# zju3dv/OnePose_Plus_Plus

Hardware: AMD Instinct MI355X
Metric: query images/sec (2D-3D match fwd) at 512x512 img x 5k pts (higher is better)
Workload: dtype f32 (operands as exact bf16 triples, f32 accumulate)

## Files before the change

onepose_plus_plus_amd/csrc/enc_layer64.hip:

```cpp
#include <stdlib.h>

#include <type_traits>

#include "enc_frag.h"

namespace {

constexpr int R64 = 64, C = 256, NW = 8, NT = 512, D = 32;
constexpr int SA = a_stride_bytes(C);
constexpr int SS = C + 4;
constexpr int OFF_S = R64 * SA, OFF_Z = OFF_S + 32 * SS * 4;
constexpr size_t kLds64 = OFF_Z + 1024;

__global__ __launch_bounds__(NT) void enc_layer64_kernel(const OppEncChain a) {
  extern __shared__ __attribute__((aligned(16))) char smem[];
  char* A = smem;
  float* S = reinterpret_cast<float*>(smem + OFF_S);
  float* z_sh = reinterpret_cast<float*>(smem + OFF_Z);

  const int tid = threadIdx.x, lane = tid & 63;
  const int wave = __builtin_amdgcn_readfirstlane(tid >> 6);
  const int half = lane >> 5, l31 = lane & 31;

  const int chunks0 = (a.len0 + R64 - 1) / R64;
  const int stream = (int)blockIdx.x >= chunks0 ? 1 : 0;
  const int cidx = stream ? blockIdx.x - chunks0 : blockIdx.x;
  const int seg_len = stream ? a.len1 : a.len0;
  const int row0 = (stream ? a.len0 : 0) + cidx * R64;
  const int nrows = min(R64, seg_len - cidx * R64);
  const float* qrows = (stream && a.q1 != nullptr) ? a.q1 + (size_t)(cidx * R64) * a.ldq : a.q + (size_t)row0 * a.ldq;

  const char* a_lane = A + l31 * SA + half * 48;
  auto gemm = [&](auto ntile_c, auto depth_c, auto s0_c, auto s1_c, auto ks_c, const void* wf, int t0, f32x16 (&acc)[2][decltype(ntile_c)::value], int tstep = 1) {
    constexpr int NTILE = decltype(ntile_c)::value, DEPTH = decltype(depth_c)::value;
    constexpr int S0 = decltype(s0_c)::value, S1 = decltype(s1_c)::value, KS = decltype(ks_c)::value;
    constexpr int NSTEP = S1 - S0;
    const __amdgpu_buffer_rsrc_t rsrc = __builtin_amdgcn_make_buffer_rsrc(const_cast<void*>(wf), 0, 0x7fffffff, 0x00020000);
    const int voff = lane * 16;
    u32x4 bq[DEPTH][NTILE][3];
    u32x4 af[2][2][3];
    auto load_b = [&](int s, int slot) {
#pragma unroll
      for (int j = 0; j < NTILE; ++j)
#pragma unroll
        for (int p = 0; p < 3; ++p)
          bq[slot][j][p] = __builtin_amdgcn_raw_buffer_load_b128(rsrc, voff, (((t0 + j * tstep) * KS + S0 + s) * 3 + p) * 1024, 0);
    };
    auto load_a = [&](int s, int slot) {
#pragma unroll
      for (int i = 0; i < 2; ++i)
#pragma unroll
        for (int q = 0; q < 3; ++q) af[slot][i][q] = *reinterpret_cast<const u32x4*>(a_lane + i * 32 * SA + s * 96 + q * 16);
    };
#pragma unroll
    for (int s = 0; s < DEPTH && s < NSTEP; ++s) load_b(s, s);
    load_a(0, 0);
    __builtin_amdgcn_sched_barrier(0);
    constexpr int PA[6] = {2, 0, 1, 1, 0, 0};
    constexpr int PB[6] = {0, 2, 1, 0, 1, 0};
#pragma unroll
    for (int s = 0; s < NSTEP; ++s) {
      if (s + 1 < NSTEP) load_a(s + 1, (s + 1) & 1);
#pragma unroll
      for (int pr = 0; pr < 6; ++pr)
#pragma unroll
        for (int i = 0; i < 2; ++i)
#pragma unroll
          for (int j = 0; j < NTILE; ++j)
            acc[i][j] = __builtin_amdgcn_mfma_f32_32x32x16_bf16(__builtin_bit_cast(bf16x8, af[s & 1][i][PA[pr]]),
                                                                 __builtin_bit_cast(bf16x8, bq[s % DEPTH][j][PB[pr]]), acc[i][j], 0, 0, 0);
      if (s + DEPTH < NSTEP) load_b(s + DEPTH, s % DEPTH);
      __builtin_amdgcn_sched_barrier(0);
    }
  };
  auto ic = [](auto v) { return v; };
  (void)ic;
  auto stage = [&](const f32x16& t, int col0, bool relu) {
#pragma unroll
    for (int r = 0; r < 16; ++r) {
      const int row = (r & 3) + 8 * (r >> 2) + 4 * half;
      float v = t[r];
      if (relu) v = v < 0.f ? 0.f : v;
      S[row * SS + col0 + l31] = v;
    }
  };
  auto split_staged = [&](int rb, int g0) {
#pragma unroll
    for (int i = 0; i < 32 * (C / 8) / NT; ++i) {
      const int p = tid + i * NT;
      const int r = p / (C / 8), g = p - r * (C / 8);
      const float4* s4 = reinterpret_cast<const float4*>(S + r * SS + g * 8);
      split8_store(s4[0], s4[1], A + (rb + r) * SA + (g0 + g) * 48);
    }
  };
  typedef float vec_t __attribute__((ext_vector_type(4)));
  auto layernorm_rows = [&](const float* gamma, const float* beta, float eps, auto mode_c, int rb) {
    constexpr int MODE = decltype(mode_c)::value;
    const vec_t gmv = *reinterpret_cast<const vec_t*>(gamma + lane * 4);
    const vec_t btv = *reinterpret_cast<const vec_t*>(beta + lane * 4);
    constexpr int RPW = 32 / NW;
    float v[RPW][4], sm[RPW], mean[RPW], rstd[RPW];
#pragma unroll
    for (int r = 0; r < RPW; ++r) {
      const vec_t t = *reinterpret_cast<const vec_t*>(S + (wave * RPW + r) * SS + lane * 4);
      sm[r] = 0.f;
#pragma unroll
      for (int i = 0; i < 4; ++i) {
        v[r][i] = t[i];
        sm[r] += t[i];
      }
    }
#pragma unroll
    for (int r = 0; r < RPW; ++r) sm[r] = opp_wave_sum_dpp(sm[r]);
#pragma unroll
    for (int r = 0; r < RPW; ++r) {
      mean[r] = sm[r] / (float)C;
      sm[r] = 0.f;
#pragma unroll
      for (int i = 0; i < 4; ++i) {
        const float d = v[r][i] - mean[r];
        sm[r] = opp_ln_sq_acc(d, sm[r]);
      }
    }
#pragma unroll
    for (int r = 0; r < RPW; ++r) sm[r] = opp_wave_sum_dpp(sm[r]);
#pragma unroll
    for (int r = 0; r < RPW; ++r) rstd[r] = 1.0f / sqrtf(sm[r] / (float)C + eps);
#pragma unroll
    for (int r = 0; r < RPW; ++r) {
      const int lr = rb + wave * RPW + r;
      float y[4];
#pragma unroll
      for (int i = 0; i < 4; ++i) y[i] = opp_ln_affine(v[r][i], mean[r], rstd[r], gmv[i], btv[i]);
      if constexpr (MODE != 0) {
        if (lr < nrows) {
          const vec_t xr = *reinterpret_cast<const vec_t*>(a.X + (size_t)(row0 + lr) * a.ldx + lane * 4);
          vec_t o;
#pragma unroll
          for (int i = 0; i < 4; ++i) o[i] = xr[i] + y[i];
          *reinterpret_cast<vec_t*>(a.out + (size_t)(row0 + lr) * a.ldo + lane * 4) = o;
#pragma unroll
          for (int i = 0; i < 4; ++i) y[i] = o[i];
        } else {
#pragma unroll
          for (int i = 0; i < 4; ++i) y[i] = 0.f;
        }
      }
      if constexpr (MODE != 1) {
        char* g = A + lr * SA + ((lane * 4) >> 3) * 48 + ((lane * 4) & 7) * 2;
#pragma unroll
        for (int i = 0; i < 4; i += 2) {
          unsigned hi, mid, lo;
          split2(y[i], y[i + 1], hi, mid, lo);
          *reinterpret_cast<unsigned*>(g + i * 2) = hi;
          *reinterpret_cast<unsigned*>(g + 16 + i * 2) = mid;
          *reinterpret_cast<unsigned*>(g + 32 + i * 2) = lo;
        }
      }
    }
  };
  auto zero2 = [](auto& acc) {
#pragma unroll
    for (auto& row : acc)
#pragma unroll
      for (auto& t : row)
#pragma unroll
        for (int r = 0; r < 16; ++r) t[r] = 0.f;
  };
  using I0 = std::integral_constant<int, 0>;
  using I1 = std::integral_constant<int, 1>;
  using I2 = std::integral_constant<int, 2>;
  using I3 = std::integral_constant<int, 3>;
  using I4 = std::integral_constant<int, 4>;
  using I16 = std::integral_constant<int, 16>;
  using I32 = std::integral_constant<int, 32>;

#pragma unroll
  for (int i = 0; i < R64 * (C / 8) / NT; ++i) {
    const int p = tid + i * NT;
    const int r = p / (C / 8), g = p - r * (C / 8);
    float4 v0 = make_float4(0.f, 0.f, 0.f, 0.f), v1 = v0;
    if (r < nrows) {
      const float4* s4 = reinterpret_cast<const float4*>(a.X + (size_t)(row0 + r) * a.ldx + g * 8);
      v0 = s4[0];
      v1 = s4[1];
    }
    split8_store(v0, v1, A + r * SA + g * 48);
  }
  const int src = a.cross ? 1 - stream : stream;
  const float src_len = (float)(src ? a.len1 : a.len0);
  const float* kvp = (src && a.kv1 != nullptr) ? a.kv1 : a.kv + (size_t)src * (C * D);
  const float* ksp = (src && a.ks1 != nullptr) ? a.ks1 : a.ks + (size_t)src * C;
  const int h = wave;
  float bk[16];
#pragma unroll
  for (int i = 0; i < 16; ++i) bk[i] = kvp[(h * D + 2 * i + half) * D + l31];
  __syncthreads();
  f32x16 hid[2][2];
  zero2(hid);
  gemm(I2{}, I3{}, I0{}, I16{}, I32{}, a.w1, wave * 2, hid);
  __syncthreads();

  constexpr int QS = 258;
  float* qsh = S;
#pragma unroll
  for (int rh = 0; rh < 2; ++rh) {
#pragma unroll
    for (int i = 0; i < 32 * (C / 4) / NT; ++i) {
      const int e = tid + i * NT;
      const int r = e / (C / 4), c4 = e - r * (C / 4);
      float4 q = make_float4(0.f, 0.f, 0.f, 0.f);
      if (rh * 32 + r < nrows) q = *reinterpret_cast<const float4*>(qrows + (size_t)(rh * 32 + r) * a.ldq + c4 * 4);
      float2* dst = reinterpret_cast<float2*>(qsh + r * QS + c4 * 4);
      dst[0] = make_float2(q.x, q.y);
      dst[1] = make_float2(q.z, q.w);
    }
    __syncthreads();
    if (tid < 8 * 32) {
      const int tok = tid & 31, hh = tid >> 5;
      const float* q = qsh + tok * QS + hh * D;
      const float* k = ksp + hh * D;
      float den = 0.f;
#pragma unroll
      for (int d = 0; d < D; ++d) den = fmaf(q[d], k[d], den);
      z_sh[hh * 32 + tok] = 1.0f / (den + a.eps_attn);
    }
    f32x16 num;
#pragma unroll
    for (int r = 0; r < 16; ++r) num[r] = 0.f;
#pragma unroll
    for (int i = 0; i < 16; ++i) num = __builtin_amdgcn_mfma_f32_32x32x2f32(qsh[l31 * QS + h * D + 2 * i + half], bk[i], num, 0, 0, 0);
    __syncthreads();
    {
      char* col = A + (h * 4 + (l31 >> 3)) * 48 + (l31 & 7) * 2;
#pragma unroll
      for (int r = 0; r < 16; ++r) {
        const int row = (r & 3) + 8 * (r >> 2) + 4 * half;
        const float v = (num[r] * z_sh[h * 32 + row]) * src_len;
        unsigned hi, mid, lo;
        split2(v, 0.f, hi, mid, lo);
        char* d = col + (rh * 32 + row) * SA;
        *reinterpret_cast<unsigned short*>(d) = (unsigned short)hi;
        *reinterpret_cast<unsigned short*>(d + 16) = (unsigned short)mid;
        *reinterpret_cast<unsigned short*>(d + 32) = (unsigned short)lo;
      }
    }
    __syncthreads();
  }

  {
    f32x16 acc[2][1];
    zero2(acc);
    gemm(I1{}, I4{}, I0{}, I16{}, I16{}, a.wm, wave, acc);
    __syncthreads();
#pragma unroll
    for (int rh = 0; rh < 2; ++rh) {
      stage(acc[rh][0], wave * 32, false);
      __syncthreads();
      layernorm_rows(a.g1, a.b1, a.eps_ln, I0{}, rh * 32);
      __syncthreads();
    }
  }

  gemm(I2{}, I3{}, I16{}, I32{}, I32{}, a.w1, wave * 2, hid);
  __syncthreads();

  f32x16 out[2][1];
  zero2(out);
#pragma unroll
  for (int kh = 0; kh < 2; ++kh) {
#pragma unroll
    for (int rh = 0; rh < 2; ++rh) {
      if (wave / (NW / 2) == kh) {
        const int c0 = (wave - kh * (NW / 2)) * 64;
        stage(hid[rh][0], c0, true);
        stage(hid[rh][1], c0 + 32, true);
      }
      __syncthreads();
      split_staged(rh * 32, 0);
      __syncthreads();
    }
    if (kh == 0) gemm(I1{}, I4{}, I0{}, I16{}, I32{}, a.w2, wave, out);
    else gemm(I1{}, I4{}, I16{}, I32{}, I32{}, a.w2, wave, out);
    __syncthreads();
  }

  const bool fold = a.wq_next != nullptr;
#pragma unroll
  for (int rh = 0; rh < 2; ++rh) {
    stage(out[rh][0], wave * 32, false);
    __syncthreads();
    if (fold) layernorm_rows(a.g2, a.b2, a.eps_ln, I2{}, rh * 32);
    else layernorm_rows(a.g2, a.b2, a.eps_ln, I1{}, rh * 32);
    __syncthreads();
  }
  if (!fold) return;

  float* qdst = (stream && a.qkv_out1 != nullptr) ? a.qkv_out1 + (size_t)(cidx * R64) * (3 * C) : a.qkv_out + (size_t)row0 * (3 * C);
  const float vdiv = (float)seg_len;
  auto finish_qkv = [&](f32x16& t, int rb, bool qk) {
#pragma unroll
    for (int r = 0; r < 16; ++r) {
      const int row = rb + (r & 3) + 8 * (r >> 2) + 4 * half;
      float v = 0.f;
      if (row < nrows) {
        v = t[r];
        if (qk) v = v > 0.f ? v + 1.f : __expf(v);
        else v = v / vdiv;
        if (stream == 0 && a.qmask != nullptr) v *= a.qmask[row0 + row];
      }
      t[r] = v;
    }
  };
  auto store_qkv = [&](const f32x16& t, int rb, int tile) {
    const int col = tile * 32 + l31;
#pragma unroll
    for (int r = 0; r < 16; ++r) {
      const int row = rb + (r & 3) + 8 * (r >> 2) + 4 * half;
      if (row < nrows) qdst[(size_t)row * (3 * C) + col] = t[r];
    }
  };
  const bool kv_fold = a.kv_part != nullptr;
  {
    f32x16 acc[2][1];
    zero2(acc);
    gemm(I1{}, I4{}, I0{}, I16{}, I16{}, a.wq_next, h, acc);
#pragma unroll
    for (int i = 0; i < 2; ++i) {
      finish_qkv(acc[i][0], i * 32, true);
      store_qkv(acc[i][0], i * 32, h);
    }
  }
  f32x16 acc[2][2];
  zero2(acc);
  gemm(I2{}, I3{}, I0{}, I16{}, I16{}, a.wq_next, NW + h, acc, NW);
#pragma unroll
  for (int i = 0; i < 2; ++i) {
    finish_qkv(acc[i][0], i * 32, true);
    finish_qkv(acc[i][1], i * 32, false);
  }
  if (!kv_fold) {
#pragma unroll
    for (int i = 0; i < 2; ++i) {
      store_qkv(acc[i][0], i * 32, NW + h);
      store_qkv(acc[i][1], i * 32, 2 * NW + h);
    }
    return;
  }
  {
    f32x16 kvacc;
#pragma unroll
    for (int r = 0; r < 16; ++r) kvacc[r] = 0.f;
    float ksum = 0.f;
    auto swap = [](float x, float y, float& lo, float& hi) {
      const auto r = __builtin_amdgcn_permlane32_swap(__builtin_bit_cast(unsigned, x), __builtin_bit_cast(unsigned, y), false, false);
      lo = __builtin_bit_cast(float, (unsigned)r[0]);
      hi = __builtin_bit_cast(float, (unsigned)r[1]);
    };
#pragma unroll
    for (int i = 0; i < 2; ++i)
#pragma unroll
      for (int q = 0; q < 4; ++q) {
        float kk[2][2], vv[2][2];
#pragma unroll
        for (int e = 0; e < 2; ++e) {
          swap(acc[i][0][4 * q + 2 * e], acc[i][0][4 * q + 2 * e + 1], kk[0][e], kk[1][e]);
          swap(acc[i][1][4 * q + 2 * e], acc[i][1][4 * q + 2 * e + 1], vv[0][e], vv[1][e]);
        }
#pragma unroll
        for (int g = 0; g < 2; ++g)
#pragma unroll
          for (int e = 0; e < 2; ++e) {
            kvacc = __builtin_amdgcn_mfma_f32_32x32x2f32(kk[g][e], vv[g][e], kvacc, 0, 0, 0);
            ksum += kk[g][e];
          }
      }
    float* kvp = a.kv_part + (size_t)blockIdx.x * (C * D) + h * (D * D);
#pragma unroll
    for (int r = 0; r < 16; ++r) {
      const int d = (r & 3) + 8 * (r >> 2) + 4 * half;
      kvp[d * D + l31] = kvacc[r];
    }
    const float tot = ksum + __shfl_xor(ksum, 32, 64);
    if (half == 0) a.ks_part[(size_t)blockIdx.x * C + h * D + l31] = tot;
  }
}

}

int opp_enc_layer64(const OppEncChain& a, hipStream_t stream) {
  OPP_CHECK_ARG(a.C == 256 && a.apply && a.X && a.out && a.q && a.kv && a.ks && a.wm && a.w1 && a.w2 && a.g1 && a.b1 && a.g2 && a.b2,
                "enc_layer64: coarse level (C = 256) with the fused attention apply only");
  OPP_CHECK_ARG(a.len0 >= 0 && a.len1 >= 0 && a.len0 + a.len1 > 0, "enc_layer64: empty token set");
  auto al16 = [](const void* p) { return (reinterpret_cast<uintptr_t>(p) & 15) == 0; };
  OPP_CHECK_ARG(al16(a.X) && al16(a.out) && al16(a.q) && a.ldx % 4 == 0 && a.ldo % 4 == 0 && a.ldq % 4 == 0 && al16(a.g1) && al16(a.b1) &&
                    al16(a.g2) && al16(a.b2) && al16(a.wm) && al16(a.w1) && al16(a.w2) && al16(a.q1), "enc_layer64: operands must be 16-byte aligned");
  OPP_CHECK_ARG(a.wq_next == nullptr || (a.qkv_out != nullptr && al16(a.wq_next)), "enc_layer64: folded projection needs its output buffer");
  OPP_CHECK_ARG((a.kv_part == nullptr) == (a.ks_part == nullptr) && (a.kv_part == nullptr || (a.wq_next != nullptr && a.qkv_out1 == nullptr)),
                "enc_layer64: the KV partials need the folded projection and both of their buffers");
  static OppLdsOnce lds_once;
  opp_lds_opt_in(reinterpret_cast<const void*>(enc_layer64_kernel), kLds64, lds_once);
  const int tiles = opp_cdiv(a.len0, R64) + opp_cdiv(a.len1, R64);
  OppProfScope prof(OPP_PROF_ENC_CHAIN, stream, 2.0 * (double)(a.len0 + a.len1) * ((a.wq_next ? 10.0 : 7.0) * C * C + 32.0 * C));
  hipLaunchKernelGGL(enc_layer64_kernel, dim3(tiles), dim3(NT), kLds64, stream, a);
  OPP_CHECK_LAUNCH("enc_layer64_kernel");
  return OPP_OK;
}
```

Baseline: 586.5.

## Keep attention message and FFN hidden in registers, cut block barriers in encoder layer

After: 586.8, median of 2. Within noise of the previous version (+0.0%).

```diff
diff --git a/onepose_plus_plus_amd/csrc/enc_layer64.hip b/onepose_plus_plus_amd/csrc/enc_layer64.hip
--- a/onepose_plus_plus_amd/csrc/enc_layer64.hip
+++ b/onepose_plus_plus_amd/csrc/enc_layer64.hip
@@ -12,7 +12,9 @@
 constexpr int OFF_S = R64 * SA, OFF_Z = OFF_S + 32 * SS * 4;
 constexpr size_t kLds64 = OFF_Z + 1024;
 
-__global__ __launch_bounds__(NT) void enc_layer64_kernel(const OppEncChain a) {
+constexpr int kStampSlots = 16, kStamps = 14;
+template <bool STAMP>
+__device__ __forceinline__ void enc_layer64_body(const OppEncChain& a, unsigned long long* ts_out) {
   extern __shared__ __attribute__((aligned(16))) char smem[];
   char* A = smem;
   float* S = reinterpret_cast<float*>(smem + OFF_S);
@@ -21,6 +23,20 @@
   const int tid = threadIdx.x, lane = tid & 63;
   const int wave = __builtin_amdgcn_readfirstlane(tid >> 6);
   const int half = lane >> 5, l31 = lane & 31;
+  unsigned long long ts[kStamps] = {};
+  auto stamp = [&](int i) {
+    if constexpr (STAMP) ts[i] = __builtin_readcyclecounter();
+  };
+  auto flush_stamps = [&]() {
+    if constexpr (STAMP) {
+      if (lane == 0) {
+        unsigned long long* o = ts_out + ((size_t)blockIdx.x * NW + wave) * kStampSlots;
+#pragma unroll
+        for (int i = 0; i < kStamps; ++i) o[i] = ts[i];
+      }
+    }
+  };
+  stamp(0);
 
   const int chunks0 = (a.len0 + R64 - 1) / R64;
   const int stream = (int)blockIdx.x >= chunks0 ? 1 : 0;
@@ -31,7 +47,7 @@
   const float* qrows = (stream && a.q1 != nullptr) ? a.q1 + (size_t)(cidx * R64) * a.ldq : a.q + (size_t)row0 * a.ldq;
 
   const char* a_lane = A + l31 * SA + half * 48;
-  auto gemm = [&](auto ntile_c, auto depth_c, auto s0_c, auto s1_c, auto ks_c, const void* wf, int t0, f32x16 (&acc)[2][decltype(ntile_c)::value], int tstep = 1) {
+  auto gemm = [&](auto ntile_c, auto depth_c, auto s0_c, auto s1_c, auto ks_c, const void* wf, int t0, f32x16 (&acc)[2][decltype(ntile_c)::value], auto&& tail, int tstep = 1) {
     constexpr int NTILE = decltype(ntile_c)::value, DEPTH = decltype(depth_c)::value;
     constexpr int S0 = decltype(s0_c)::value, S1 = decltype(s1_c)::value, KS = decltype(ks_c)::value;
     constexpr int NSTEP = S1 - S0;
@@ -70,30 +86,51 @@
             acc[i][j] = __builtin_amdgcn_mfma_f32_32x32x16_bf16(__builtin_bit_cast(bf16x8, af[s & 1][i][PA[pr]]),
                                                                  __builtin_bit_cast(bf16x8, bq[s % DEPTH][j][PB[pr]]), acc[i][j], 0, 0, 0);
       if (s + DEPTH < NSTEP) load_b(s + DEPTH, s % DEPTH);
+      if (s + DEPTH == NSTEP) tail();
       __builtin_amdgcn_sched_barrier(0);
     }
   };
-  auto ic = [](auto v) { return v; };
-  (void)ic;
-  auto stage = [&](const f32x16& t, int col0, bool relu) {
+  auto none = [] {};
+  auto stage = [&](const f32x16& t, int col0) {
 #pragma unroll
     for (int r = 0; r < 16; ++r) {
       const int row = (r & 3) + 8 * (r >> 2) + 4 * half;
-      float v = t[r];
-      if (relu) v = v < 0.f ? 0.f : v;
-      S[row * SS + col0 + l31] = v;
-    }
-  };
-  auto split_staged = [&](int rb, int g0) {
-#pragma unroll
-    for (int i = 0; i < 32 * (C / 8) / NT; ++i) {
-      const int p = tid + i * NT;
-      const int r = p / (C / 8), g = p - r * (C / 8);
-      const float4* s4 = reinterpret_cast<const float4*>(S + r * SS + g * 8);
-      split8_store(s4[0], s4[1], A + (rb + r) * SA + (g0 + g) * 48);
-    }
+      S[row * SS + col0 + l31] = t[r];
+    }
+  };
+  auto acc_to_operand = [&](const f32x16& t, int rb, int c0) {
+    const int odd = l31 & 1;
+    char* base = A + (rb + 4 * half + odd) * SA + ((c0 + l31) >> 3) * 48 + (l31 & 6) * 2;
+#pragma unroll
+    for (int r = 0; r < 16; r += 2) {
+      const float e = t[r], o = t[r + 1];
+      const float got = __builtin_bit_cast(float, __builtin_amdgcn_update_dpp(0, __builtin_bit_cast(int, odd ? +e : +o), 0xB1, 0xF, 0xF, true));
+      unsigned hi, mid, lo;
+      split2(odd ? +got : +e, odd ? +o : +got, hi, mid, lo);
+      char* d = base + ((r & 3) + 8 * (r >> 2)) * SA;
+      *reinterpret_cast<unsigned*>(d) = hi;
+      *reinterpret_cast<unsigned*>(d + 16) = mid;
+      *reinterpret_cast<unsigned*>(d + 32) = lo;
+    }
+  };
+  auto relu16 = [](const f32x16& t) {
+    f32x16 o;
+#pragma unroll
+    for (int r = 0; r < 16; ++r) o[r] = t[r] < 0.f ? 0.f : t[r];
+    return o;
   };
   typedef float vec_t __attribute__((ext_vector_type(4)));
+  vec_t xres[2][32 / NW];
+  auto load_x_rows = [&]() {
+#pragma unroll
+    for (int rh = 0; rh < 2; ++rh)
+#pragma unroll
+      for (int r = 0; r < 32 / NW; ++r) {
+        const int lr = rh * 32 + wave * (32 / NW) + r;
+        xres[rh][r] = vec_t{0.f, 0.f, 0.f, 0.f};
+        if (lr < nrows) xres[rh][r] = *reinterpret_cast<const vec_t*>(a.X + (size_t)(row0 + lr) * a.ldx + lane * 4);
+      }
+  };
   auto layernorm_rows = [&](const float* gamma, const float* beta, float eps, auto mode_c, int rb) {
     constexpr int MODE = decltype(mode_c)::value;
     const vec_t gmv = *reinterpret_cast<const vec_t*>(gamma + lane * 4);
@@ -134,7 +171,7 @@
       for (int i = 0; i < 4; ++i) y[i] = opp_ln_affine(v[r][i], mean[r], rstd[r], gmv[i], btv[i]);
       if constexpr (MODE != 0) {
         if (lr < nrows) {
-          const vec_t xr = *reinterpret_cast<const vec_t*>(a.X + (size_t)(row0 + lr) * a.ldx + lane * 4);
+          const vec_t xr = xres[rb / 32][r];
           vec_t o;
 #pragma unroll
           for (int i = 0; i < 4; ++i) o[i] = xr[i] + y[i];
@@ -175,17 +212,24 @@
   using I16 = std::integral_constant<int, 16>;
   using I32 = std::integral_constant<int, 32>;
 
-#pragma unroll
-  for (int i = 0; i < R64 * (C / 8) / NT; ++i) {
-    const int p = tid + i * NT;
-    const int r = p / (C / 8), g = p - r * (C / 8);
-    float4 v0 = make_float4(0.f, 0.f, 0.f, 0.f), v1 = v0;
-    if (r < nrows) {
-      const float4* s4 = reinterpret_cast<const float4*>(a.X + (size_t)(row0 + r) * a.ldx + g * 8);
-      v0 = s4[0];
-      v1 = s4[1];
-    }
-    split8_store(v0, v1, A + r * SA + g * 48);
+  {
+    constexpr int XI = R64 * (C / 8) / NT;
+    float4 xv[XI][2];
+#pragma unroll
+    for (int i = 0; i < XI; ++i) {
+      const int p = tid + i * NT;
+      const int r = p / (C / 8), g = p - r * (C / 8);
+      const float4* s4 = reinterpret_cast<const float4*>(a.X + (size_t)(row0 + min(r, nrows - 1)) * a.ldx + g * 8);
+      xv[i][0] = s4[0];
+      xv[i][1] = s4[1];
+    }
+#pragma unroll
+    for (int i = 0; i < XI; ++i) {
+      const int p = tid + i * NT;
+      const int r = p / (C / 8), g = p - r * (C / 8);
+      const float4 zero = make_float4(0.f, 0.f, 0.f, 0.f);
+      split8_store(r < nrows ? xv[i][0] : zero, r < nrows ? xv[i][1] : zero, A + r * SA + g * 48);
+    }
   }
   const int src = a.cross ? 1 - stream : stream;
   const float src_len = (float)(src ? a.len1 : a.len0);
@@ -196,105 +240,116 @@
 #pragma unroll
   for (int i = 0; i < 16; ++i) bk[i] = kvp[(h * D + 2 * i + half) * D + l31];
   __syncthreads();
+  stamp(1);
+  auto load_q = [&](int rh, float4 (&q)[8]) {
+    const float4* p = reinterpret_cast<const float4*>(qrows + (size_t)min(rh * 32 + l31, nrows - 1) * a.ldq + h * D);
+#pragma unroll
+    for (int i = 0; i < 8; ++i) q[i] = p[i];
+  };
+  float4 qv0[8];
   f32x16 hid[2][2];
   zero2(hid);
-  gemm(I2{}, I3{}, I0{}, I16{}, I32{}, a.w1, wave * 2, hid);
+  gemm(I2{}, I3{}, I0{}, I16{}, I32{}, a.w1, wave * 2, hid, [&] { load_q(0, qv0); });
   __syncthreads();
-
-  constexpr int QS = 258;
-  float* qsh = S;
+  stamp(2);
+
+  float4 qv1[8];
+  load_q(1, qv1);
 #pragma unroll
   for (int rh = 0; rh < 2; ++rh) {
-#pragma unroll
-    for (int i = 0; i < 32 * (C / 4) / NT; ++i) {
-      const int e = tid + i * NT;
-      const int r = e / (C / 4), c4 = e - r * (C / 4);
-      float4 q = make_float4(0.f, 0.f, 0.f, 0.f);
-      if (rh * 32 + r < nrows) q = *reinterpret_cast<const float4*>(qrows + (size_t)(rh * 32 + r) * a.ldq + c4 * 4);
-      float2* dst = reinterpret_cast<float2*>(qsh + r * QS + c4 * 4);
-      dst[0] = make_float2(q.x, q.y);
-      dst[1] = make_float2(q.z, q.w);
-    }
-    __syncthreads();
-    if (tid < 8 * 32) {
-      const int tok = tid & 31, hh = tid >> 5;
-      const float* q = qsh + tok * QS + hh * D;
-      const float* k = ksp + hh * D;
+    float q[D];
+#pragma unroll
+    for (int i = 0; i < 8; ++i) {
+      float4 t = qv0[i];
+      if (rh) t = qv1[i];
+      if (rh * 32 + l31 >= nrows) t = make_float4(0.f, 0.f, 0.f, 0.f);
+      q[4 * i] = t.x, q[4 * i + 1] = t.y, q[4 * i + 2] = t.z, q[4 * i + 3] = t.w;
+    }
+    {
+      const float* k = ksp + h * D;
       float den = 0.f;
 #pragma unroll
       for (int d = 0; d < D; ++d) den = fmaf(q[d], k[d], den);
-      z_sh[hh * 32 + tok] = 1.0f / (den + a.eps_attn);
-    }
+      z_sh[h * 32 + l31] = 1.0f / (den + a.eps_attn);
+    }
+    __builtin_amdgcn_fence(__ATOMIC_RELEASE, "wavefront");
+    __builtin_amdgcn_wave_barrier();
+    __builtin_amdgcn_fence(__ATOMIC_ACQUIRE, "wavefront");
     f32x16 num;
 #pragma unroll
     for (int r = 0; r < 16; ++r) num[r] = 0.f;
 #pragma unroll
-    for (int i = 0; i < 16; ++i) num = __builtin_amdgcn_mfma_f32_32x32x2f32(qsh[l31 * QS + h * D + 2 * i + half], bk[i], num, 0, 0, 0);
-    __syncthreads();
-    {
-      char* col = A + (h * 4 + (l31 >> 3)) * 48 + (l31 & 7) * 2;
-#pragma unroll
-      for (int r = 0; r < 16; ++r) {
-        const int row = (r & 3) + 8 * (r >> 2) + 4 * half;
-        const float v = (num[r] * z_sh[h * 32 + row]) * src_len;
-        unsigned hi, mid, lo;
-        split2(v, 0.f, hi, mid, lo);
-        char* d = col + (rh * 32 + row) * SA;
-        *reinterpret_cast<unsigned short*>(d) = (unsigned short)hi;
-        *reinterpret_cast<unsigned short*>(d + 16) = (unsigned short)mid;
-        *reinterpret_cast<unsigned short*>(d + 32) = (unsigned short)lo;
-      }
-    }
-    __syncthreads();
-  }
+    for (int i = 0; i < 16; ++i) {
+      const float qe = q[2 * i], qo = q[2 * i + 1];
+      num = __builtin_amdgcn_mfma_f32_32x32x2f32(half ? +qo : +qe, bk[i], num, 0, 0, 0);
+    }
+    f32x16 msg;
+#pragma unroll
+    for (int r = 0; r < 16; ++r) msg[r] = (num[r] * z_sh[h * 32 + (r & 3) + 8 * (r >> 2) + 4 * half]) * src_len;
+    acc_to_operand(msg, rh * 32, h * 32);
+    __builtin_amdgcn_fence(__ATOMIC_RELEASE, "wavefront");
+    __builtin_amdgcn_wave_barrier();
+  }
+  __syncthreads();
+  stamp(3);
 
   {
     f32x16 acc[2][1];
     zero2(acc);
-    gemm(I1{}, I4{}, I0{}, I16{}, I16{}, a.wm, wave, acc);
-    __syncthreads();
+    gemm(I1{}, I4{}, I0{}, I16{}, I16{}, a.wm, wave, acc, none);
+    stamp(4);
 #pragma unroll
     for (int rh = 0; rh < 2; ++rh) {
-      stage(acc[rh][0], wave * 32, false);
+      stage(acc[rh][0], wave * 32);
       __syncthreads();
       layernorm_rows(a.g1, a.b1, a.eps_ln, I0{}, rh * 32);
       __syncthreads();
     }
   }
-
-  gemm(I2{}, I3{}, I16{}, I32{}, I32{}, a.w1, wave * 2, hid);
+  stamp(5);
+
+  gemm(I2{}, I3{}, I16{}, I32{}, I32{}, a.w1, wave * 2, hid, none);
   __syncthreads();
+  stamp(6);
 
   f32x16 out[2][1];
   zero2(out);
 #pragma unroll
   for (int kh = 0; kh < 2; ++kh) {
-#pragma unroll
-    for (int rh = 0; rh < 2; ++rh) {
-      if (wave / (NW / 2) == kh) {
-        const int c0 = (wave - kh * (NW / 2)) * 64;
-        stage(hid[rh][0], c0, true);
-        stage(hid[rh][1], c0 + 32, true);
-      }
+    if (wave / (NW / 2) == kh) {
+      const int c0 = (wave - kh * (NW / 2)) * 64;
+#pragma unroll
+      for (int rh = 0; rh < 2; ++rh) {
+        acc_to_operand(relu16(hid[rh][0]), rh * 32, c0);
+        acc_to_operand(relu16(hid[rh][1]), rh * 32, c0 + 32);
+      }
+    }
+    __syncthreads();
+    stamp(7 + 2 * kh);
+    if (kh == 0) {
+      gemm(I1{}, I4{}, I0{}, I16{}, I32{}, a.w2, wave, out, none);
       __syncthreads();
-      split_staged(rh * 32, 0);
-      __syncthreads();
-    }
-    if (kh == 0) gemm(I1{}, I4{}, I0{}, I16{}, I32{}, a.w2, wave, out);
-    else gemm(I1{}, I4{}, I16{}, I32{}, I32{}, a.w2, wave, out);
-    __syncthreads();
+    } else {
+      load_x_rows();
+      gemm(I1{}, I4{}, I16{}, I32{}, I32{}, a.w2, wave, out, none);
+    }
+    stamp(8 + 2 * kh);
   }
 
   const bool fold = a.wq_next != nullptr;
 #pragma unroll
   for (int rh = 0; rh < 2; ++rh) {
-    stage(out[rh][0], wave * 32, false);
+    stage(out[rh][0], wave * 32);
     __syncthreads();
     if (fold) layernorm_rows(a.g2, a.b2, a.eps_ln, I2{}, rh * 32);
     else layernorm_rows(a.g2, a.b2, a.eps_ln, I1{}, rh * 32);
     __syncthreads();
   }
-  if (!fold) return;
+  stamp(11);
+  if (!fold) {
+    flush_stamps();
+    return;
+  }
 
   float* qdst = (stream && a.qkv_out1 != nullptr) ? a.qkv_out1 + (size_t)(cidx * R64) * (3 * C) : a.qkv_out + (size_t)row0 * (3 * C);
   const float vdiv = (float)seg_len;
@@ -324,7 +379,7 @@
   {
     f32x16 acc[2][1];
     zero2(acc);
-    gemm(I1{}, I4{}, I0{}, I16{}, I16{}, a.wq_next, h, acc);
+    gemm(I1{}, I4{}, I0{}, I16{}, I16{}, a.wq_next, h, acc, none);
 #pragma unroll
     for (int i = 0; i < 2; ++i) {
       finish_qkv(acc[i][0], i * 32, true);
@@ -333,18 +388,20 @@
   }
   f32x16 acc[2][2];
   zero2(acc);
-  gemm(I2{}, I3{}, I0{}, I16{}, I16{}, a.wq_next, NW + h, acc, NW);
+  gemm(I2{}, I3{}, I0{}, I16{}, I16{}, a.wq_next, NW + h, acc, none, NW);
 #pragma unroll
   for (int i = 0; i < 2; ++i) {
     finish_qkv(acc[i][0], i * 32, true);
     finish_qkv(acc[i][1], i * 32, false);
   }
+  stamp(12);
   if (!kv_fold) {
 #pragma unroll
     for (int i = 0; i < 2; ++i) {
       store_qkv(acc[i][0], i * 32, NW + h);
       store_qkv(acc[i][1], i * 32, 2 * NW + h);
     }
+    flush_stamps();
     return;
   }
   {
@@ -384,7 +441,18 @@
     const float tot = ksum + __shfl_xor(ksum, 32, 64);
     if (half == 0) a.ks_part[(size_t)blockIdx.x * C + h * D + l31] = tot;
   }
+  stamp(13);
+  flush_stamps();
 }
+
+__global__ __launch_bounds__(NT) void enc_layer64_kernel(const OppEncChain a) { enc_layer64_body<false>(a, nullptr); }
+
+#ifdef OPP_TUNING
+__global__ __launch_bounds__(NT) void enc_layer64_stamped_kernel(const OppEncChain a, unsigned long long* ts) { enc_layer64_body<true>(a, ts); }
+unsigned long long* g_enc64_ts = nullptr;
+int g_enc64_ts_launches = 0, g_enc64_ts_done = 0;
+size_t g_enc64_ts_used = 0;
+#endif
 
 }
 
@@ -402,7 +470,28 @@
   opp_lds_opt_in(reinterpret_cast<const void*>(enc_layer64_kernel), kLds64, lds_once);
   const int tiles = opp_cdiv(a.len0, R64) + opp_cdiv(a.len1, R64);
   OppProfScope prof(OPP_PROF_ENC_CHAIN, stream, 2.0 * (double)(a.len0 + a.len1) * ((a.wq_next ? 10.0 : 7.0) * C * C + 32.0 * C));
+#ifdef OPP_TUNING
+  if (g_enc64_ts != nullptr && g_enc64_ts_done < g_enc64_ts_launches) {
+    static OppLdsOnce lds_once_stamped;
+    opp_lds_opt_in(reinterpret_cast<const void*>(enc_layer64_stamped_kernel), kLds64, lds_once_stamped);
+    hipLaunchKernelGGL(enc_layer64_stamped_kernel, dim3(tiles), dim3(NT), kLds64, stream, a, g_enc64_ts + g_enc64_ts_used);
+    OPP_CHECK_LAUNCH("enc_layer64_stamped_kernel");
+    g_enc64_ts_used += (size_t)tiles * NW * kStampSlots;
+    ++g_enc64_ts_done;
+    return OPP_OK;
+  }
+#endif
   hipLaunchKernelGGL(enc_layer64_kernel, dim3(tiles), dim3(NT), kLds64, stream, a);
   OPP_CHECK_LAUNCH("enc_layer64_kernel");
   return OPP_OK;
 }
+
+#ifdef OPP_TUNING
+extern "C" int opp_enc64_phase_stamps(void* buf, int launches) {
+  g_enc64_ts = static_cast<unsigned long long*>(buf);
+  g_enc64_ts_launches = buf ? launches : 0;
+  g_enc64_ts_done = 0;
+  g_enc64_ts_used = 0;
+  return OPP_OK;
+}
+#endif
```
